# jaak-s/BayesianDataFusion.jl

Hardware: AMD Instinct MI355X
Metric: Gibbs sweeps/sec (both entities) + test RMSE, MovieLens-1M D=32 (higher is better)
Workload: dtype f64; 1 GPU; BPMF MovieLens-1M 6040x3952, 500209 training ratings (500000 held out), D=32, alpha=1.5, step = rows of both entities + hyperpriors + test prediction update (one native call); BEFORE the --warmup steps the engine's set-up runs 60 ms of full iterations whose results are discarded (device_warmup_ms); num_latent=32, burnin=5, psamples=1985, parallelism=1 GPU

## Files before the change

bayesiandatafusion.jl_amd/csrc/bdf_common.h:

```cpp
#pragma once
#include <map>
#include <array>
#include <algorithm>
#include <numeric>
#include <hip/hip_runtime.h>
#include <hip/hip_ext.h>
#include <cstdint>
#include <cstdio>
#include <cstdarg>
#include <cstring>
#include <vector>
#include "../../include/bdf.h"

void bdf_set_error(const char *fmt, ...);

#define BDF_HIP(expr)                                                                      \
    do {                                                                                   \
        hipError_t e__ = (expr);                                                           \
        if (e__ != hipSuccess) {                                                           \
            bdf_set_error("%s failed: %s (%s:%d)", #expr, hipGetErrorString(e__), __FILE__, __LINE__); \
            return BDF_ERR_HIP;                                                            \
        }                                                                                  \
    } while (0)

// ... 77 lines not shown
    bdf_rows_state *rows;
    double *norm_part;
};

int bdf_scratch(bdf_ctx *ctx, size_t bytes, void **out);
int bdf_scratch2(bdf_ctx *ctx, size_t bytes, void **out);
int bdf_sum_ranks_into(bdf_ctx *ctx, bdf_comm *comm, double *x, int64_t n, double *gather);
int bdf_sample_beta_rel_impl(bdf_ctx *ctx, bdf_comm *comm, const bdf_feat *fc, const bdf_pairs *train, int64_t first_obs, int D,
                             const double *const *factors, double mean_value, double alpha, const double *alpha_dev, double lambda_beta,
                             uint32_t rel_tag, double *beta_out, double *linear_out, double *rhs_out);
#define BDF_DRAWS_BATCH 8
int bdf_hyper_draws_batch(bdf_ctx *ctx, int D, int n, const int64_t *N, const double *nu, const uint32_t *entity_tag, double *const *draws_out);

struct bdf_mode_index {
    std::vector<int64_t> rowptr;
    std::vector<int64_t> rowids;
    std::vector<int32_t> order;
    int64_t *rowptr_dev;
    int32_t *colidx_dev;
    double  *vals_dev;
    int32_t *perm_dev;
    uint32_t *packed_dev;
    int32_t *order_dev;
    std::vector<int32_t> own_orig;
    std::vector<int32_t> own_pos;
    std::vector<int64_t> own_q;
    std::vector<int64_t> chunk_begin;
    int64_t own_nnz;
};

struct bdf_rel {
    bdf_ctx *ctx;
    uint64_t serial;
    int n_modes;
    int64_t dims[BDF_MAX_MODES];
    int64_t nnz;
    double value_mean;
    bdf_mode_index idx[BDF_MAX_MODES];
    int sharded;
    int rank, world, chunks;
    int64_t nint[BDF_MAX_MODES];
    int n_codes;
    double *table_dev;
};

struct bdf_pairs {
    bdf_ctx *ctx;
    int n_modes;
    int64_t n;
    int32_t *ids_dev;
    double *values_dev;
    double *avg_dev, *sq_dev;
    double count;
    const double *baseline_dev;
    int32_t *orig_dev;
    int sorted_mode;
    std::vector<int32_t> ids_host, orig_host;
    std::vector<double> values_host;
    void *auc_ws;
    int link;
    double link_r;
    double *lpd_dev;
    double lpd_draws;
    double *waic_dev;
    double waic_draws;
};

#define BDF_ORD_TABLE 17
#define BDF_ORD_CUR 0
#define BDF_ORD_PROP 17
#define BDF_ORD_JAC 34
#define BDF_ORD_SIGMA 35
#define BDF_ORD_PROPOSALS 36
#define BDF_ORD_ACCEPTS 37
#define BDF_ORD_LAST_S 38
#define BDF_ORD_ACCEPTED 39
#define BDF_ORD_VALID 40
#define BDF_ORD_LOGU 41
#define BDF_ORD_TRACE 48
#define BDF_ORD_MAX_TRACE ((int64_t)1 << 24)
struct bdf_ordinal {
    bdf_ctx *ctx;
    int K;
    int64_t capacity;
    int64_t adapt_steps;
    size_t state_doubles;
    double *state_dev;
    hipStream_t stream;
};

struct bdf_feat {
    bdf_ctx *ctx;
    int kind;
    int64_t m, n, nnz;
    double *dense_dev;
    int64_t *rowptr_dev; int32_t *colind_dev; double *rvals_dev;
    int64_t *colptr_dev; int32_t *rowind_dev; double *cvals_dev;
    int64_t *panel_fwd_dev; int n_panels_fwd;
    int64_t *panel_tr_dev; int n_panels_tr;
    double *FF_dev;
    int32_t *row_ids_dev;
    double *chol_ws;
    size_t chol_ws_doubles;
    void *gather_dev;
    size_t gather_bytes;
    bdf_feat *eig_Q;
    double *eig_s;
    double *eig_y;
    int eig_y_cols;
    bool eig_failed;
    bool FF_summed;
};
#define BDF_EIG_MAX 640

int bdf_chol_solve(bdf_ctx *ctx, bdf_feat *f, int D, const double *lambda_dev, const double *rhs, double *beta);

struct u32x4 { uint32_t x, y, z, w; };

__host__ __device__ __forceinline__ u32x4 philox4x32_10(u32x4 c, uint32_t k0, uint32_t k1)
{
#pragma unroll
    for (int r = 0; r < 10; r++) {
        uint64_t p0 = (uint64_t)0xD2511F53u * c.x;
        uint64_t p1 = (uint64_t)0xCD9E8D57u * c.z;
        u32x4 n;
        n.x = (uint32_t)(p1 >> 32) ^ c.y ^ k0;
        n.y = (uint32_t)p1;
        n.z = (uint32_t)(p0 >> 32) ^ c.w ^ k1;
        n.w = (uint32_t)p0;
        c = n;
        k0 += 0x9E3779B9u;
        k1 += 0xBB67AE85u;
    }
    return c;
}

__host__ __device__ __forceinline__ u32x4 bdf_draw(uint64_t seed, uint32_t sweep, uint32_t purpose, uint32_t entity,
                                          uint64_t row, uint32_t pair)
{
    u32x4 c;
    c.x = (uint32_t)row;
    c.y = (uint32_t)((row >> 32) & 0xffffu) | (pair << 16);
    c.z = sweep;
    c.w = (purpose << 24) | (entity & 0xffffffu);
    return philox4x32_10(c, (uint32_t)seed, (uint32_t)(seed >> 32));
}

__host__ __device__ __forceinline__ double bdf_u01(uint32_t lo, uint32_t hi)
{
    uint64_t x = ((uint64_t)hi << 32) | lo;
    return ((double)(x >> 11) + 0.5) * 0x1.0p-53;
}

__device__ __forceinline__ void bdf_sincos2pi(double u, double &s, double &c)
{
    const double q = rint(4.0 * u);
    const double x = 6.283185307179586476925286766559 * fma(q, -0.25, u);
    const double z = x * x;
    const double ps = fma(z, fma(z, fma(z, fma(z, fma(z, 1.58969099521155010221e-10, -2.50507602534068634195e-08),
                                                   2.75573137070700676789e-06), -1.98412698298579493134e-04),
                                     8.33333333332248946124e-03), -1.66666666666666324348e-01);
    const double pc = fma(z, fma(z, fma(z, fma(z, fma(z, -1.13596475577881948265e-11, 2.08757232129817482790e-09),
                                                   -2.75573143513906633035e-07), 2.48015872894767294178e-05),
                                     -1.38888888888741095749e-03), 4.16666666666666019037e-02);
    const double sx = fma(x * z, ps, x);
    const double cx = fma(z * z, pc, fma(z, -0.5, 1.0));
    const int iq = (int)q & 3;
    const double sa = (iq & 1) ? cx : sx, ca = (iq & 1) ? sx : cx;
    s = (iq & 2) ? -sa : sa;
    c = (iq == 1 || iq == 2) ? -ca : ca;
}

__device__ __forceinline__ double bdf_log01(double x)
{
    int k;
    double m = frexp(x, &k);
    if (m < 0.70710678118654752440) { m *= 2.0; k -= 1; }
    const double f = m - 1.0, dk = (double)k;
    const double s = f / (2.0 + f), z = s * s, w = z * z;
    const double t1 = w * fma(w, fma(w, 1.531383769920937332e-01, 2.222219843214978396e-01), 3.999999999940941908e-01);
    const double t2 = z * fma(w, fma(w, fma(w, 1.479819860511658591e-01, 1.818357216161805012e-01), 2.857142874366239149e-01),
                              6.666666666666735130e-01);
    const double R = t2 + t1, hfsq = 0.5 * f * f;
    return dk * 6.93147180369123816490e-01 - ((hfsq - fma(s, hfsq + R, dk * 1.90821492927058770002e-10)) - f);
}

__device__ __forceinline__ double bdf_normal(uint64_t seed, uint32_t sweep, uint32_t purpose, uint32_t entity,
                                    uint64_t row, int n)
{
    u32x4 o = bdf_draw(seed, sweep, purpose, entity, row, (uint32_t)(n >> 1));
    double u1 = bdf_u01(o.x, o.y), u2 = bdf_u01(o.z, o.w);
    double r = sqrt(-2.0 * bdf_log01(u1));
    double s, c;
    bdf_sincos2pi(u2, s, c);
    return (n & 1) ? r * s : r * c;
}

__device__ __forceinline__ void bdf_normal_pair(uint64_t seed, uint32_t sweep, uint32_t purpose, uint32_t entity,
                                       uint64_t row, uint32_t pair, double &z0, double &z1)
{
    u32x4 o = bdf_draw(seed, sweep, purpose, entity, row, pair);
    double u1 = bdf_u01(o.x, o.y), u2 = bdf_u01(o.z, o.w);
    double r = sqrt(-2.0 * bdf_log01(u1));
    double s, c;
    bdf_sincos2pi(u2, s, c);
    z0 = r * c;
    z1 = r * s;
}

__device__ __forceinline__ double bdf_uniform(uint64_t seed, uint32_t sweep, uint32_t purpose, uint32_t entity,
                                     uint64_t row, uint32_t pair)
{
    u32x4 o = bdf_draw(seed, sweep, purpose, entity, row, pair);
    return bdf_u01(o.x, o.y);
}

__device__ __forceinline__ double bdf_gamma_on(uint32_t p_normal, uint32_t p_uniform, uint64_t seed, uint32_t sweep, uint32_t entity,
                                               uint64_t g, double a)
{
    double boost = 1.0;
    if (a < 1.0) {
        boost = pow(bdf_uniform(seed, sweep, p_uniform, entity, g, 0xffffu), 1.0 / a);
        a += 1.0;
    }
    double d = a - 1.0 / 3.0, c = 1.0 / sqrt(9.0 * d);
    for (uint32_t t = 0; t < 256; t++) {
        double x = bdf_normal(seed, sweep, p_normal, entity, g, (int)(2 * t));
        double v = 1.0 + c * x;
        if (v <= 0.0) continue;
        v = v * v * v;
        double u = bdf_uniform(seed, sweep, p_uniform, entity, g, t);
        if (u < 1.0 - 0.0331 * (x * x) * (x * x)) return boost * d * v;
        if (log(u) < 0.5 * x * x + d * (1.0 - v + log(v))) return boost * d * v;
    }
    return boost * d;
}

__device__ __forceinline__ double bdf_gamma(uint64_t seed, uint32_t sweep, uint32_t entity, uint64_t g, double a)
{
    return bdf_gamma_on(BDF_P_GAMMA_N, BDF_P_GAMMA_U, seed, sweep, entity, g, a);
}

__device__ __forceinline__ double readlane_f64(double v, int lane)
{
    int lo = __builtin_amdgcn_readlane(__double2loint(v), lane);
    int hi = __builtin_amdgcn_readlane(__double2hiint(v), lane);
    return __hiloint2double(hi, lo);
}

#define BDF_DONE_SHARDS 64
#define BDF_DONE_STRIDE 16

int bdf_predict_plain(bdf_ctx *ctx, const bdf_pairs *p, int D, const double *const *factors, double mean_value, double *out);
int bdf_predict_link(bdf_ctx *ctx, const bdf_pairs *p, int D, const double *const *factors, double mean_value, const double *linear,
                     double *out, int phase, double count, double clamp_lo, double clamp_hi, double class_cut, double *stats_out);
int bdf_predict_link_pg(bdf_ctx *ctx, const bdf_pairs *p, int D, const double *const *factors, double mean_value, const double *linear,
                        double *out, int phase, double count, double clamp_lo, double clamp_hi, double class_cut, double *stats_out);
```

bayesiandatafusion.jl_amd/csrc/k_predict.hip:

```cpp
#include "bdf_common.h"
#include "predict.h"
#include <algorithm>
#include <cstdlib>

namespace {

template <int NM, int VEC, int NC>
__global__ __launch_bounds__(256) void k_predict(PredArgs a)
{
    const int tid = threadIdx.x, sub = tid & 7;
    double st[4] = {0.0, 0.0, 0.0, 0.0};
    const int64_t ngroups = (int64_t)gridDim.x * 32, ntrips = (a.n + 7) / 8;
    constexpr int BATCH = (VEC == 1) ? 2 : (NC * NM <= 3 ? 4 : 2);
    for (int64_t trip = (int64_t)blockIdx.x * 32 + tid / 8; trip < ntrips; trip += ngroups) {
        const int64_t p0 = trip * 8;
        PairState ps;
        pair_load(a, p0 + sub, ps);
        int32_t my[NM];
#pragma unroll
        for (int k = 0; k < NM; k++) my[k] = a.ids[(int64_t)k * a.n + ps.pm];
        double keep = 0.0;
#pragma unroll
        for (int u0 = 0; u0 < 8; u0 += BATCH) {
            if (p0 + u0 >= a.n) break;
// ... 134 lines not shown
}

namespace {
struct PredAllArgs {
    int D, n_modes;
    int64_t dims[BDF_MAX_MODES];
    const double *fac[BDF_MAX_MODES];
    double mean;
    double *out;
    int64_t rest;
};
__global__ __launch_bounds__(256) void k_predict_all(PredAllArgs a)
{
    __shared__ double u[16][BDF_MAX_D + 1];
    const int tx = threadIdx.x & 15, ty = threadIdx.x >> 4;
    const int64_t i0 = (int64_t)blockIdx.y * 16, c = (int64_t)blockIdx.x * 16 + tx;
    for (int e = threadIdx.x; e < 16 * a.D; e += 256) {
        const int r = e / a.D, d = e - r * a.D;
        u[r][d] = i0 + r < a.dims[0] ? a.fac[0][(i0 + r) * a.D + d] : 0.0;
    }
    __syncthreads();
    if (c >= a.rest || i0 + ty >= a.dims[0]) return;
    const double *row[BDF_MAX_MODES];
    int64_t q = c;
#pragma unroll
    for (int k = BDF_MAX_MODES - 1; k >= 1; k--)
        if (k < a.n_modes) { row[k] = a.fac[k] + (q % a.dims[k]) * a.D; q /= a.dims[k]; }
    double s = 0.0;
    for (int d = 0; d < a.D; d++) {
        double pr = u[ty][d];
#pragma unroll
        for (int k = 1; k < BDF_MAX_MODES; k++)
            if (k < a.n_modes) pr *= row[k][d];
        s += pr;
    }
    a.out[(i0 + ty) * a.rest + c] = s + a.mean;
}
}

extern "C" int bdf_predict_all(bdf_ctx *ctx, int n_modes, const int64_t *dims, int D, const double *const *factors,
                               double mean_value, double *out)
{
    BDF_REQUIRE(ctx && dims && factors && out, BDF_ERR_ARG, "bdf_predict_all: NULL argument");
    BDF_REQUIRE(n_modes >= 2 && n_modes <= BDF_MAX_MODES, BDF_ERR_ARG, "bdf_predict_all: n_modes=%d must be in 2..%d", n_modes, BDF_MAX_MODES);
    BDF_REQUIRE(D >= 1 && D <= BDF_MAX_D, BDF_ERR_ARG, "bdf_predict_all: num_latent=%d must be in 1..%d", D, BDF_MAX_D);
    PredAllArgs a;
    memset(&a, 0, sizeof(a));
    a.D = D; a.n_modes = n_modes; a.mean = mean_value; a.out = out; a.rest = 1;
    for (int k = 0; k < n_modes; k++) {
        BDF_REQUIRE(dims[k] >= 0 && factors[k] != nullptr, BDF_ERR_ARG, "bdf_predict_all: dims[%d] < 0 or factors[%d] NULL", k, k);
        a.dims[k] = dims[k]; a.fac[k] = factors[k];
        if (k >= 1) a.rest *= dims[k];
    }
    if (a.dims[0] == 0 || a.rest == 0) return BDF_OK;
    const int64_t gx = (a.rest + 15) / 16, gy = (a.dims[0] + 15) / 16;
    BDF_REQUIRE(gx < (int64_t)0x7fffffff && gy <= 65535 * (int64_t)1024, BDF_ERR_BOUNDS, "bdf_predict_all: %lld x %lld cells are too many for one launch",
                (long long)a.dims[0], (long long)a.rest);
    BDF_HIP(hipSetDevice(ctx->device));
    for (int64_t y0 = 0; y0 < gy; y0 += 65535) {
        PredAllArgs b = a;
        const int64_t ny = std::min<int64_t>(65535, gy - y0);
        b.fac[0] = a.fac[0] + y0 * 16 * D;
        b.dims[0] = std::min<int64_t>(a.dims[0] - y0 * 16, ny * 16);
        b.out = a.out + y0 * 16 * a.rest;
        hipLaunchKernelGGL(k_predict_all, dim3((unsigned)gx, (unsigned)ny), dim3(256), 0, ctx->stream, b);
    }
    BDF_HIP(hipGetLastError());
    return BDF_OK;
}

extern "C" int bdf_pairs_create(bdf_ctx *ctx, int n_modes, int64_t n, const void *ids, int id_bytes,
                                const double *values, bdf_pairs **out)
{
    BDF_REQUIRE(ctx && out, BDF_ERR_ARG, "bdf_pairs_create: NULL argument");
    BDF_REQUIRE(n_modes >= 2 && n_modes <= BDF_MAX_MODES, BDF_ERR_ARG, "bdf_pairs_create: n_modes=%d must be in 2..%d", n_modes, BDF_MAX_MODES);
    BDF_REQUIRE(id_bytes == 4 || id_bytes == 8, BDF_ERR_ARG, "bdf_pairs_create: id_bytes must be 4 or 8");
    BDF_REQUIRE(n >= 0 && (n == 0 || (ids && values)), BDF_ERR_ARG, "bdf_pairs_create: ids/values NULL");
    BDF_HIP(hipSetDevice(ctx->device));
    std::vector<int32_t> h((size_t)n * n_modes);
    for (size_t q = 0; q < h.size(); q++) {
        int64_t v = id_bytes == 8 ? ((const int64_t *)ids)[q] : (int64_t)((const int32_t *)ids)[q];
        BDF_REQUIRE(v >= 1 && v < (int64_t)0x7fffffff, BDF_ERR_BOUNDS, "bdf_pairs_create: id %lld out of range", (long long)v);
        h[q] = (int32_t)(v - 1);
    }
    bdf_pairs *p = new bdf_pairs();
    p->ctx = ctx; p->n_modes = n_modes; p->n = n; p->count = 0.0; p->baseline_dev = nullptr; p->orig_dev = nullptr; p->sorted_mode = -1;
    p->ids_dev = nullptr; p->values_dev = nullptr; p->avg_dev = nullptr; p->sq_dev = nullptr; p->auc_ws = nullptr; p->link = 0; p->link_r = 0.0;
    p->lpd_dev = nullptr; p->lpd_draws = 0.0; p->waic_dev = nullptr; p->waic_draws = 0.0;
    struct Guard { bdf_pairs *p; ~Guard() { if (p) bdf_pairs_destroy(p); } } guard{p};
    p->ids_host = h;
    p->values_host.assign(values, values + (n ? n : 0));
    size_t nb = std::max<size_t>((size_t)n * sizeof(double), 8);
    BDF_HIP(hipMalloc((void **)&p->ids_dev, std::max<size_t>(h.size() * sizeof(int32_t), 8)));
    BDF_HIP(hipMalloc((void **)&p->values_dev, nb));
    BDF_HIP(hipMalloc((void **)&p->avg_dev, nb));
    BDF_HIP(hipMalloc((void **)&p->sq_dev, nb));
    if (n) {
        BDF_HIP(hipMemcpy(p->ids_dev, h.data(), h.size() * sizeof(int32_t), hipMemcpyHostToDevice));
        BDF_HIP(hipMemcpy(p->values_dev, values, (size_t)n * sizeof(double), hipMemcpyHostToDevice));
    }
    BDF_HIP(hipMemsetAsync(p->avg_dev, 0, nb, ctx->stream));
    BDF_HIP(hipMemsetAsync(p->sq_dev, 0, nb, ctx->stream));
    BDF_HIP(hipStreamSynchronize(ctx->stream));
    guard.p = nullptr;
    *out = p;
    return BDF_OK;
}

extern "C" int bdf_pairs_destroy(bdf_pairs *p)
{
    if (!p) return BDF_OK;
    hipSetDevice(p->ctx->device);
    hipStreamSynchronize(p->ctx->stream);
    hipFree(p->ids_dev); hipFree(p->values_dev); hipFree(p->avg_dev); hipFree(p->sq_dev);
    if (p->orig_dev) hipFree(p->orig_dev);
    if (p->auc_ws) hipFree(p->auc_ws);
    if (p->lpd_dev) hipFree(p->lpd_dev);
    if (p->waic_dev) hipFree(p->waic_dev);
    delete p;
    return BDF_OK;
}

extern "C" int bdf_predict(bdf_ctx *ctx, const bdf_pairs *p, int D, const double *const *factors,
                           double mean_value, double *out)
{
    PredArgs a;
    int rc = fill("bdf_predict", ctx, p, D, factors, a);
    if (rc) return rc;
    BDF_REQUIRE(out != nullptr, BDF_ERR_ARG, "bdf_predict: out is NULL");
    a.mean = mean_value; a.out = out;
    return p->link ? bdf_predict_link(ctx, p, D, factors, mean_value, nullptr, out, -1, 0.0, 1.0, 0.0, 0.0, nullptr) : launch_predict(ctx, a);
}

int bdf_predict_plain(bdf_ctx *ctx, const bdf_pairs *p, int D, const double *const *factors, double mean_value, double *out)
{
    PredArgs a;
    int rc = fill("bdf_predict", ctx, p, D, factors, a);
    if (rc) return rc;
    a.mean = mean_value; a.linear = nullptr; a.out = out;
    return launch_predict(ctx, a);
}

extern "C" int bdf_predict_update(bdf_ctx *ctx, bdf_pairs *p, int D, const double *const *factors,
                                  double mean_value, int phase, double clamp_lo, double clamp_hi,
                                  double class_cut, double *stats_out)
{
    PredArgs a;
    int rc = fill("bdf_predict_update", ctx, p, D, factors, a);
    if (rc) return rc;
    BDF_REQUIRE(stats_out != nullptr, BDF_ERR_ARG, "bdf_predict_update: stats_out is NULL");
    BDF_REQUIRE(phase >= 0 && phase <= 2, BDF_ERR_ARG, "bdf_predict_update: phase must be 0, 1 or 2");
    a.mean = mean_value; a.avg = p->avg_dev; a.sq = p->sq_dev; a.phase = phase; a.count = p->count;
    a.clamp_lo = clamp_lo; a.clamp_hi = clamp_hi; a.cut = class_cut; a.stats = stats_out;
    rc = p->link ? bdf_predict_link(ctx, p, D, factors, mean_value, nullptr, nullptr, phase, p->count, clamp_lo, clamp_hi, class_cut, stats_out)
                 : launch_predict(ctx, a);
    if (rc) return rc;
    if (phase == 1) p->count = 1.0;
    else if (phase == 2) p->count += 1.0;
    return BDF_OK;
}

extern "C" int bdf_predict_sse(bdf_ctx *ctx, const bdf_pairs *p, int D, const double *const *factors, double mean_value,
                               const double *linear_values, double *stats_out)
{
    PredArgs a;
    int rc = fill("bdf_predict_sse", ctx, p, D, factors, a);
    if (rc) return rc;
    BDF_REQUIRE(stats_out != nullptr, BDF_ERR_ARG, "bdf_predict_sse: stats_out is NULL");
    a.mean = mean_value; if (linear_values) a.linear = linear_values; a.phase = 3; a.count = 0.0;
    a.clamp_lo = 1.0; a.clamp_hi = 0.0; a.cut = 0.0; a.stats = stats_out;
    if (p->link) return bdf_predict_link(ctx, p, D, factors, mean_value, linear_values, nullptr, 3, 0.0, 1.0, 0.0, 0.0, stats_out);
    return launch_predict(ctx, a);
}

extern "C" int bdf_pairs_sort(bdf_pairs *p, int mode)
{
    BDF_REQUIRE(p != nullptr, BDF_ERR_ARG, "bdf_pairs_sort: NULL argument");
    BDF_REQUIRE(mode >= 0 && mode < p->n_modes, BDF_ERR_ARG, "bdf_pairs_sort: mode %d out of range", mode);
    BDF_REQUIRE(p->count == 0.0 && p->orig_dev == nullptr, BDF_ERR_ARG, "bdf_pairs_sort: the pairs already hold prediction state or are sorted");
    const int64_t n = p->n;
    if (n == 0) return BDF_OK;
    BDF_HIP(hipSetDevice(p->ctx->device));
    std::vector<int32_t> perm((size_t)n);
    for (int64_t i = 0; i < n; i++) perm[(size_t)i] = (int32_t)i;
    const int32_t *key = p->ids_host.data() + (size_t)mode * n;
    std::stable_sort(perm.begin(), perm.end(), [key](int32_t x, int32_t y) { return key[x] < key[y]; });
    std::vector<int32_t> ids((size_t)n * p->n_modes);
    std::vector<double> vals((size_t)n);
    for (int k = 0; k < p->n_modes; k++)
        for (int64_t i = 0; i < n; i++) ids[(size_t)k * n + i] = p->ids_host[(size_t)k * n + perm[(size_t)i]];
    for (int64_t i = 0; i < n; i++) vals[(size_t)i] = p->values_host[(size_t)perm[(size_t)i]];
    BDF_HIP(hipStreamSynchronize(p->ctx->stream));
    BDF_HIP(hipMemcpy(p->ids_dev, ids.data(), ids.size() * sizeof(int32_t), hipMemcpyHostToDevice));
    BDF_HIP(hipMemcpy(p->values_dev, vals.data(), vals.size() * sizeof(double), hipMemcpyHostToDevice));
    BDF_HIP(hipMalloc((void **)&p->orig_dev, (size_t)n * sizeof(int32_t)));
    BDF_HIP(hipMemcpy(p->orig_dev, perm.data(), (size_t)n * sizeof(int32_t), hipMemcpyHostToDevice));
    p->orig_host = perm;
    p->sorted_mode = mode;
    return BDF_OK;
}

extern "C" int bdf_pairs_order(const bdf_pairs *p, int64_t *orig_host)
{
    BDF_REQUIRE(p && orig_host, BDF_ERR_ARG, "bdf_pairs_order: NULL argument");
    for (int64_t i = 0; i < p->n; i++) orig_host[i] = p->orig_host.empty() ? i : (int64_t)p->orig_host[(size_t)i];
    return BDF_OK;
}

extern "C" int bdf_pairs_set_baseline(bdf_pairs *p, const double *baseline)
{
    BDF_REQUIRE(p != nullptr, BDF_ERR_ARG, "bdf_pairs_set_baseline: NULL argument");
    p->baseline_dev = baseline;
    return BDF_OK;
}

extern "C" int bdf_pairs_set_link(bdf_pairs *p, int link)
{
    BDF_REQUIRE(p != nullptr, BDF_ERR_ARG, "bdf_pairs_set_link: NULL argument");
    BDF_REQUIRE(link == 0 || link == 1, BDF_ERR_ARG, "bdf_pairs_set_link: link=%d must be 0 (identity) or 1 (probit)", link);
    p->link = link;
    return BDF_OK;
}

extern "C" int bdf_pairs_set_logistic_link(bdf_pairs *p)
{
    BDF_REQUIRE(p != nullptr, BDF_ERR_ARG, "bdf_pairs_set_logistic_link: NULL argument");
    p->link = 2;
    return BDF_OK;
}

extern "C" int bdf_pairs_set_count_link(bdf_pairs *p, double r)
{
    BDF_REQUIRE(p != nullptr, BDF_ERR_ARG, "bdf_pairs_set_count_link: NULL argument");
    BDF_REQUIRE(r >= 1.0 && r <= 2147483648.0 && r == std::floor(r), BDF_ERR_ARG, "bdf_pairs_set_count_link: r=%g must be an integer, at least 1", r);
    p->link = 3;
    p->link_r = r;
    return BDF_OK;
}

extern "C" int bdf_pairs_state(const bdf_pairs *p, double **avg, double **sq, int64_t *n)
{
    BDF_REQUIRE(p && avg && sq && n, BDF_ERR_ARG, "bdf_pairs_state: NULL argument");
    *avg = p->avg_dev; *sq = p->sq_dev; *n = p->n;
    return BDF_OK;
}
```

bayesiandatafusion.jl_amd/csrc/k_rows_col.hip:

```cpp
#include "rows.h"
#include "dpp_rows32.h"
#include <algorithm>

#ifndef BDF_COL_WAVES
#define BDF_COL_WAVES 2
#endif
#define COL_PSZ 800

#ifdef BDF_K1_STAMPS
#define CSTAMP_DECL unsigned long long st_t = __builtin_amdgcn_s_memtime(), st_acc = 0, st_mid = 0, st_prior = 0, st_fin = 0, st_rng = 0, st_steps = 0, st_rounds = 0, st_parts = 0, st_fins = 0, st_folds = 0; const unsigned long long st_begin = st_t
#define CSTAMP(x) do { const unsigned long long now_ = __builtin_amdgcn_s_memtime(); x += now_ - st_t; st_t = now_; } while (0)
#else
#define CSTAMP_DECL do { } while (0)
#define CSTAMP(x) do { } while (0)
#endif

namespace {

template <int DR, int K>
__device__ __forceinline__ void col_obs(double (&A0)[33], double (&A1)[33], double v0, double v1, double r)
{
    col_rank1<DR, 0>(A0, A1, v0, v1);
    fm1_run<K>(A0[32], r, v0);
    fm1_run<K>(A1[32], r, v1);
}

__device__ __forceinline__ double col_ld(__amdgpu_buffer_rsrc_t rs, uint32_t off)
{
    typedef unsigned u2v __attribute__((ext_vector_type(2)));
    const u2v x = __builtin_amdgcn_raw_buffer_load_b64(rs, (int)off, 0, 0);
    return __hiloint2double((int)x.y, (int)x.x);
}

template <bool FULL, int K0>
__device__ __forceinline__ void col_gather4(double (&b)[4][2], __amdgpu_buffer_rsrc_t rs, uint32_t idw, uint32_t rowb, uint32_t eo, bool ok1)
{
#pragma unroll
    for (int q = 0; q < 4; q++) {
        uint32_t id;
        if (q == 0) id = row_bcast_u32<K0>(idw); else if (q == 1) id = row_bcast_u32<K0 + 1>(idw);
        else if (q == 2) id = row_bcast_u32<K0 + 2>(idw); else id = row_bcast_u32<K0 + 3>(idw);
        if constexpr (FULL) {
            const uint32_t base = id + eo;
            b[q][1] = col_ld(rs, base);
            b[q][0] = col_ld(rs, base + 128u);
        } else {
            const uint32_t base = id + eo;
            b[q][0] = col_ld(rs, base);
            b[q][1] = col_ld(rs, ok1 ? base - 128u : 0xffffffffu);
        }
    }
}
template <int DR, int K0>
__device__ __forceinline__ void col_compute4(double (&A0)[33], double (&A1)[33], const double (&b)[4][2], double r)
{
    col_obs<DR, K0>(A0, A1, b[0][0], b[0][1], r);
    col_obs<DR, K0 + 1>(A0, A1, b[1][0], b[1][1], r);
    col_obs<DR, K0 + 2>(A0, A1, b[2][0], b[2][1], r);
    col_obs<DR, K0 + 3>(A0, A1, b[3][0], b[3][1], r);
}

template <int X>
__device__ __forceinline__ void col_fold(double (&A0)[33], double (&A1)[33], double m)
{
#pragma unroll
    for (int i = 0; i < 33; i++) A0[i] = fma(__shfl_xor(A0[i], X), m, A0[i]);
#pragma unroll
    for (int i = 16; i < 33; i++) A1[i] = fma(__shfl_xor(A1[i], X), m, A1[i]);
}

template <int E0, int E1, bool ADD>
__device__ __forceinline__ void col_slot_load(double (&A0)[33], double (&A1)[33], const double *src, double m)
{
#pragma unroll
    for (int e = E0; e < E1; e++) {
        const double v = src[e * 16];
        double &d = e < 33 ? A0[e] : A1[e - 17];
        if (ADD) d = fma(v, m, d); else d = v * m;
    }
}

__device__ __forceinline__ void col_prior_dma(const double *image, unsigned lds_dst, int lane)
{
    const void *sbase = (const void *)(((uint64_t)(uint32_t)__builtin_amdgcn_readfirstlane((int)((uint64_t)image >> 32)) << 32) |
                                       (uint32_t)__builtin_amdgcn_readfirstlane((int)(uint32_t)(uint64_t)image));
#pragma unroll
    for (int k = 0; k < 6; k++) {
        const unsigned voff = (unsigned)k * 1024u + (unsigned)lane * 16u;
        unsigned keep;
        asm volatile("s_mov_b32 %0, m0\n\ts_mov_b32 m0, %2\n\ts_nop 0\n\tglobal_load_lds_dwordx4 %1, %3 sc1\n\ts_mov_b32 m0, %0"
                     : "=&s"(keep) : "v"(voff), "s"(lds_dst + (unsigned)k * 1024u), "s"(sbase) : "memory");
    }
}
template <int S, int I, int DR>
__device__ __forceinline__ void col_prior_lds(double (&A)[33], const double *img, double alpha, int j)
{
    if constexpr (I < DR) {
        A[I] = fma(alpha, A[I], img[sys_off<S, I>(j)]);
        col_prior_lds<S, I + 1, DR>(A, img, alpha, j);
    }
}

template <int DR, bool FULL>
__global__ __launch_bounds__(64, BDF_COL_WAVES) void k_rows_col(SampleArgs a_in, ColPlanDev p_in, uint32_t fac_bytes)
{
    __shared__ __attribute__((aligned(16))) double lds[4 * 272 + 768];
    const int w = blockIdx.x;
    if (w >= p_in.n_waves) return;
    const int r_end = p_in.wave_round[w + 1];
    if (a_in.span && threadIdx.x == 0) atomicMin(a_in.span + 2 * (w & 63), (unsigned long long)__builtin_amdgcn_s_memrealtime());
    CSTAMP_DECL;
#pragma nounroll
    for (int rd = p_in.wave_round[w]; rd < r_end; rd++) {
    int zero = 0, lane = threadIdx.x;
    asm volatile("" : "+s"(zero), "+v"(lane));
    const SampleArgs &a = (&a_in)[zero];
    const ColPlanDev &p = (&p_in)[zero];
    const int j = lane & 15, g = lane >> 4;
    const TermDev &T = a.t[0];
    const int D = FULL ? 32 : a.D;
    const int ec0 = D - 1 - j, ec1 = D - 17 - j;
    const int n0 = ec0, n1 = ec1 >= 0 ? ec1 : 0;
    const bool ok1 = ec1 >= 0;
    const uint32_t rowb = (uint32_t)D * 8u;
    const uint32_t eo = FULL ? (uint32_t)ec1 * 8u : (uint32_t)ec0 * 8u;
    const __amdgpu_buffer_rsrc_t rs = __builtin_amdgcn_make_buffer_rsrc((void *)T.fac[0], 0, (int)fac_bytes, 0x00020000);
    const bool coded = T.packed != nullptr;
    const double mean = T.mean;
    {
        const ColJob jb = p.jobs[(int64_t)rd * 4 + g];
        const bool live = jb.row >= 0;
        const int n = live ? jb.count : 0;
        const unsigned lds_img = (unsigned)__builtin_amdgcn_readfirstlane((int)(unsigned)(size_t)(__attribute__((address_space(3))) double *)(lds + 4 * 272));
        bool have_prior = true;
        if (a.ready) have_prior = __builtin_amdgcn_readfirstlane((int)((int32_t)(__hip_atomic_load(a.ready, __ATOMIC_RELAXED, __HIP_MEMORY_SCOPE_AGENT) - a.ready_want) >= 0)) != 0;
        if (have_prior) col_prior_dma(a.prior_c, lds_img, lane);
        double A0[33], A1[33];
#pragma unroll
        for (int i = 0; i < 33; i++) { A0[i] = 0.0; A1[i] = 0.0; }
        int nmax = n;
        nmax = max(nmax, __shfl_xor(nmax, 16));
        nmax = max(nmax, __shfl_xor(nmax, 32));
        nmax = __builtin_amdgcn_readfirstlane(nmax);
        if (nmax > 0) {
            const uint32_t *packed = coded ? T.packed + jb.q_begin : nullptr;
            const int32_t *colidx = T.colidx + jb.q_begin;
            const double *vals = T.vals + jb.q_begin;
            const double *table = T.table;
#define COL_CHUNK(c0, IDW, R)                                                                     \
            {                                                                                     \
                const int o_ = (c0) + j;                                                          \
                IDW = 0xffffffu; R = 0.0;                                                         \
                if (o_ < n) {                                                                     \
                    if (coded) { const uint32_t pw_ = packed[o_]; IDW = pw_; R = table[pw_ >> 24] - mean; } \
                    else { IDW = (uint32_t)colidx[o_]; R = vals[o_] - mean; }                     \
                }                                                                                 \
                IDW = __umul24(IDW, rowb);       \
            }
            uint32_t idw_c, idw_n;
            double r_c, r_n;
            COL_CHUNK(0, idw_c, r_c)
            double ba[4][2], bb[4][2];
            col_gather4<FULL, 0>(ba, rs, idw_c, rowb, eo, ok1);
            for (int c0 = 0;; c0 += 16) {
                COL_CHUNK(c0 + 16, idw_n, r_n)
                col_gather4<FULL, 4>(bb, rs, idw_c, rowb, eo, ok1);
                __builtin_amdgcn_sched_barrier(0);
                col_compute4<DR, 0>(A0, A1, ba, r_c);
                if (c0 + 4 >= nmax) break;
                col_gather4<FULL, 8>(ba, rs, idw_c, rowb, eo, ok1);
                __builtin_amdgcn_sched_barrier(0);
                col_compute4<DR, 4>(A0, A1, bb, r_c);
                if (c0 + 8 >= nmax) break;
                col_gather4<FULL, 12>(bb, rs, idw_c, rowb, eo, ok1);
                __builtin_amdgcn_sched_barrier(0);
                col_compute4<DR, 8>(A0, A1, ba, r_c);
                if (c0 + 12 >= nmax) break;
                col_gather4<FULL, 0>(ba, rs, idw_n, rowb, eo, ok1);
                __builtin_amdgcn_sched_barrier(0);
                col_compute4<DR, 12>(A0, A1, bb, r_c);
                if (c0 + 16 >= nmax) break;
                idw_c = idw_n; r_c = r_n;
            }
#undef COL_CHUNK
        }
#ifdef BDF_K1_STAMPS
        asm volatile("s_nop 0" :: "v"(A0[0]), "v"(A0[32]), "v"(A1[31]));
        st_steps += (unsigned long long)nmax; st_rounds++;
#endif
        CSTAMP(st_acc);
        const unsigned fl = (unsigned)jb.flags;
        if (__builtin_amdgcn_readfirstlane((int)(__ballot((fl & COLF_PAIR) != 0) != 0ull))) {
#ifdef BDF_K1_STAMPS
            st_folds++;
#endif
            col_fold<16>(A0, A1, (fl & COLF_PAIR) ? 1.0 : 0.0);
            if (__builtin_amdgcn_readfirstlane((int)(__ballot((fl & COLF_QUAD) != 0) != 0ull)))
                col_fold<32>(A0, A1, (fl & COLF_QUAD) ? 1.0 : 0.0);
        }
        if (__builtin_amdgcn_readfirstlane((int)(fl & COLF_MULTI))) {
            const int srow = __builtin_amdgcn_readfirstlane(jb.srow);
            double *dst = p.partials + (int64_t)__builtin_amdgcn_readfirstlane(jb.slot) * COL_PSZ + j;
            if (g == 0) {
#pragma unroll
                for (int e = 0; e < 33; e++) __hip_atomic_store(dst + e * 16, A0[e], __ATOMIC_RELAXED, __HIP_MEMORY_SCOPE_AGENT);
#pragma unroll
                for (int e = 33; e < 50; e++) __hip_atomic_store(dst + e * 16, A1[e - 17], __ATOMIC_RELAXED, __HIP_MEMORY_SCOPE_AGENT);
            }
            const ColSplit sr = p.rows[srow];
            asm volatile("s_waitcnt vmcnt(0)" ::: "memory");
            int old = 0;
            if (lane == 0) old = __hip_atomic_fetch_add(p.arrived + srow, 1, __ATOMIC_RELAXED, __HIP_MEMORY_SCOPE_AGENT);
            old = __builtin_amdgcn_readfirstlane(old);
#ifdef BDF_K1_STAMPS
            st_parts++;
            if (old == sr.n_slots - 1) st_fins++;
#endif
            if (old != sr.n_slots - 1) { CSTAMP(st_mid); continue; }
            __builtin_amdgcn_fence(__ATOMIC_ACQUIRE, "agent");
            asm volatile("s_waitcnt vmcnt(0)" ::: "memory");
            if (lane == 0) p.arrived[srow] = 0;
            const double *src = p.partials + (int64_t)sr.slot_begin * COL_PSZ + j;
            col_slot_load<0, 50, false>(A0, A1, src + (int64_t)(g < sr.n_slots ? g : 0) * COL_PSZ, g < sr.n_slots ? 1.0 : 0.0);
            for (int s0 = 4; s0 < sr.n_slots; s0 += 4) {
                const bool on = s0 + g < sr.n_slots;
                const double *sp = src + (int64_t)(on ? s0 + g : 0) * COL_PSZ;
                const double m = on ? 1.0 : 0.0;
                col_slot_load<0, 16, true>(A0, A1, sp, m);
                asm volatile("" ::: "memory");
                col_slot_load<16, 33, true>(A0, A1, sp, m);
                asm volatile("" ::: "memory");
                col_slot_load<33, 50, true>(A0, A1, sp, m);
                asm volatile("" ::: "memory");
            }
            col_fold<16>(A0, A1, 1.0);
            col_fold<32>(A0, A1, 1.0);
        }
        CSTAMP(st_mid);
        double z0 = 0.0, z1 = 0.0;
        {
            double ze = 0.0, zo = 0.0;
            if (live && 2 * j < D) bdf_normal_pair(a.seed, a.sweep, BDF_P_ROW, a.entity_tag, (uint64_t)(uint32_t)jb.orig, (uint32_t)j, ze, zo);
            const int base = lane & 48;
            const double ze0 = __shfl(ze, base + (n0 >> 1)), zo0 = __shfl(zo, base + (n0 >> 1));
            const double ze1 = __shfl(ze, base + (n1 >> 1)), zo1 = __shfl(zo, base + (n1 >> 1));
            z0 = (n0 & 1) ? zo0 : ze0;
            z1 = ok1 ? ((n1 & 1) ? zo1 : ze1) : 0.0;
        }
        asm volatile("" ::: "memory");
        CSTAMP(st_rng);
        {
            double *tl = lds + g * 272;
#pragma unroll
            for (int r = 0; r < 16; r++) tl[r * 17 + j] = A0[16 + r];
            wave_sync();
#pragma unroll
            for (int i = 0; i < 16; i++) A1[i] = tl[j * 17 + i];
            wave_sync();
        }
        CSTAMP(st_mid);
        const double alpha = term_alpha(T);
        if (!have_prior) {
            int spins = 0;
            while ((int32_t)(__hip_atomic_load(a.ready, __ATOMIC_RELAXED, __HIP_MEMORY_SCOPE_AGENT) - a.ready_want) < 0) {
                __builtin_amdgcn_s_sleep(16);
                if (++spins > (1 << 22)) { if (lane == 0) atomicOr_system(a.flag, 16); break; }
            }
            col_prior_dma(a.prior_c, lds_img, lane);
        }
        {
            const double *pb = a.prior_b + (a.mu_is_matrix && live ? (int64_t)jb.row * D : 0);
            const double b0 = __hip_atomic_load(pb + n0, __ATOMIC_RELAXED, __HIP_MEMORY_SCOPE_AGENT);
            const double b1 = __hip_atomic_load(pb + n1, __ATOMIC_RELAXED, __HIP_MEMORY_SCOPE_AGENT);
            asm volatile("s_waitcnt vmcnt(0)" ::: "memory");
            wave_sync();
            const double *img = lds + 4 * 272;
            col_prior_lds<0, 0, DR>(A0, img, alpha, j);
            col_prior_lds<1, 0, DR>(A1, img, alpha, j);
            A0[32] = fma(alpha, A0[32], b0);
            A1[32] = ok1 ? fma(alpha, A1[32], b1) : 0.0;
            wave_sync();
        }
#ifdef BDF_K1_STAMPS
        asm volatile("s_nop 0" :: "v"(A0[0]), "v"(A0[31]), "v"(A1[0]), "v"(A1[31]));
#endif
        CSTAMP(st_prior);
        double d0 = 1.0, d1 = 1.0;
        fin_factor<DR, 0>(A0, A1, d0, d1, j);
        const bool lead = live && (fl & COLF_LEADER);
        if (lead && (!(d0 > 0.0) || (ok1 && !(d1 > 0.0)))) atomicOr_system(a.flag, 1);
        const double rd0 = fast_rcp(d0), rd1 = fast_rcp(d1);
        double y0 = fma(z0, fast_rsqrt(d0), A0[32] * rd0), y1 = fma(z1, fast_rsqrt(d1), A1[32] * rd1);
        fin_backward<DR - 1>(A0, A1, y0, y1, rd0, rd1, j);
        if (lead) __hip_atomic_store(a.out + ((int64_t)jb.row * D + ec0), y0, __ATOMIC_RELAXED, __HIP_MEMORY_SCOPE_AGENT);
        if (lead && ok1) __hip_atomic_store(a.out + ((int64_t)jb.row * D + ec1), y1, __ATOMIC_RELAXED, __HIP_MEMORY_SCOPE_AGENT);
        CSTAMP(st_fin);
    }
    }
    if (a_in.done) {
        asm volatile("s_waitcnt vmcnt(0)" ::: "memory");
        if (threadIdx.x == 0) __hip_atomic_fetch_add(a_in.done + BDF_DONE_STRIDE * (w & (BDF_DONE_SHARDS - 1)), 1u, __ATOMIC_RELAXED, __HIP_MEMORY_SCOPE_AGENT);
    }
    if (a_in.span && threadIdx.x == 0) atomicMax(a_in.span + 2 * (w & 63) + 1, (unsigned long long)__builtin_amdgcn_s_memrealtime());
#ifdef BDF_K1_STAMPS
    if (threadIdx.x == 0 && a_in.b_dump && w < 65536) {
        unsigned long long *d = (unsigned long long *)a_in.b_dump + (size_t)w * 16;
        d[0] = st_begin; d[8] = st_t; d[6] = st_rounds; d[7] = st_steps;
        d[1] = st_parts; d[2] = st_fins; d[3] = st_folds;
        d[11] = st_rng; d[12] = st_acc; d[13] = st_mid; d[14] = st_prior; d[15] = st_fin;
        d[9] = __builtin_amdgcn_s_getreg((4 - 1) << 11 | 0 << 6 | 4) | ((unsigned long long)__builtin_amdgcn_s_getreg((32 - 1) << 11 | 0 << 6 | 4));
        d[10] = __builtin_amdgcn_s_getreg((4 - 1) << 11 | 0 << 6 | 20);
    }
#endif
}

#define COL_C_OBS 56.0
#define COL_C_FIN 1460.0
#define COL_C_FOLD 180.0
#define COL_C_PART 700.0

struct Round { ColJob job[4]; double cost; };

ColJob idle_job() { return ColJob{-1, 0, 0, 0, -1, 0, 0}; }

}

int bdf_col_plan_build(bdf_ctx *ctx, const std::vector<bdf_row_ref> &rows, int T, int64_t slots, bdf_col_plan &plan)
{
    std::vector<Round> rounds;
    std::vector<ColSplit> splits;
    struct Unit { int32_t row, orig; int64_t qb; int32_t n; };
    std::vector<Unit> singles, pairs;
    int32_t n_slots_total = 0;
    auto quad_round = [&](const bdf_row_ref &rr, int64_t b0, int64_t b1, int32_t srow, int32_t slot, double fin_share) {
        Round R;
        const int64_t m = b1 - b0;
        int32_t lmax = 0;
        for (int q = 0; q < 4; q++) {
            const int64_t p0 = b0 + m * q / 4, p1 = b0 + m * (q + 1) / 4;
            R.job[q] = ColJob{rr.out, rr.orig, rr.qb + p0, (int32_t)(p1 - p0), srow, slot,
                              (int32_t)(COLF_PAIR | COLF_QUAD | (q == 0 ? COLF_LEADER : 0) | (srow >= 0 ? COLF_MULTI : 0))};
            lmax = std::max(lmax, (int32_t)(p1 - p0));
        }
        constexpr double part_extra = 3000.0;
        R.cost = COL_C_OBS * lmax + 2 * COL_C_FOLD + (srow >= 0 ? COL_C_PART + fin_share + part_extra : COL_C_FIN);
        rounds.push_back(R);
    };
    for (const bdf_row_ref &rr : rows) {
        const int64_t n = rr.cnt;
        if (n <= T) singles.push_back(Unit{rr.out, rr.orig, rr.qb, (int32_t)n});
        else if (n <= 2 * (int64_t)T) pairs.push_back(Unit{rr.out, rr.orig, rr.qb, (int32_t)n});
        else if (n <= 4 * (int64_t)T) quad_round(rr, 0, n, -1, 0, 0.0);
        else {
            const int64_t W = (n + 4 * (int64_t)T - 1) / (4 * (int64_t)T);
            BDF_REQUIRE(W < (1 << 20), BDF_ERR_ARG, "bdf_sample_rows: a row of %lld observations", (long long)n);
            const int32_t srow = (int32_t)splits.size();
            splits.push_back(ColSplit{n_slots_total, (int32_t)W});
            const double share = (COL_C_FIN + 2 * COL_C_FOLD + 60.0 * (double)((W + 3) / 4)) / (double)W;
            for (int64_t q = 0; q < W; q++) quad_round(rr, n * q / W, n * (q + 1) / W, srow, n_slots_total + (int32_t)q, share);
            n_slots_total += (int32_t)W;
        }
    }
    auto by_len = [](const Unit &x, const Unit &y) { return x.n > y.n; };
    std::stable_sort(pairs.begin(), pairs.end(), by_len);
    std::stable_sort(singles.begin(), singles.end(), by_len);
    auto pair_jobs = [](const Unit &u, ColJob *dst) {
        const int32_t h = u.n / 2;
        dst[0] = ColJob{u.row, u.orig, u.qb, h, -1, 0, COLF_PAIR | COLF_LEADER};
        dst[1] = ColJob{u.row, u.orig, u.qb + h, u.n - h, -1, 0, COLF_PAIR};
    };
    size_t si = 0;
    for (size_t pi = 0; pi < pairs.size(); pi += 2) {
        Round R;
        pair_jobs(pairs[pi], R.job);
        int32_t lmax = pairs[pi].n - pairs[pi].n / 2;
        if (pi + 1 < pairs.size()) pair_jobs(pairs[pi + 1], R.job + 2);
        else {
            for (int q = 2; q < 4; q++) {
                if (si < singles.size()) {
                    const Unit &u = singles[si++];
                    R.job[q] = ColJob{u.row, u.orig, u.qb, u.n, -1, 0, COLF_LEADER};
                    lmax = std::max(lmax, u.n);
                } else R.job[q] = idle_job();
            }
        }
        R.cost = COL_C_OBS * lmax + COL_C_FOLD + COL_C_FIN;
        rounds.push_back(R);
    }
    for (; si < singles.size(); si += 4) {
        Round R;
        for (int q = 0; q < 4; q++) {
            if (si + q < singles.size()) {
                const Unit &u = singles[si + q];
                R.job[q] = ColJob{u.row, u.orig, u.qb, u.n, -1, 0, COLF_LEADER};
            } else R.job[q] = idle_job();
// ... 80 lines not shown
```

Before: 12310 sweeps/s.

## Add sorted-run test prediction kernel and cap column-kernel VGPRs with SGPR constants

Adds a new prediction-update kernel for sorted two-mode test pairs. Each 8-lane group handles a run of 16 consecutive pairs and reloads the sorted-side factor row only when its id changes, which cuts redundant gathers. Separately, the row-sampling column kernel gets an explicit VGPR cap, and its RNG polynomial constants are forced into scalar registers through a template coefficient policy, to relieve vector register pressure. The cap risks spills, and the new path assumes sorted ids with D a multiple of 4 and at most 32.

Measured after the change: 12740 sweeps/s (median of 6 runs). +3.4%, better.

```diff
diff --git a/bayesiandatafusion.jl_amd/csrc/bdf_common.h b/bayesiandatafusion.jl_amd/csrc/bdf_common.h
--- a/bayesiandatafusion.jl_amd/csrc/bdf_common.h
+++ b/bayesiandatafusion.jl_amd/csrc/bdf_common.h
@@ -253,17 +253,20 @@
     return ((double)(x >> 11) + 0.5) * 0x1.0p-53;
 }
 
+struct BdfLiteral { static __device__ __forceinline__ double c(double x) { return x; } };
+
+template <class KC = BdfLiteral>
 __device__ __forceinline__ void bdf_sincos2pi(double u, double &s, double &c)
 {
     const double q = rint(4.0 * u);
-    const double x = 6.283185307179586476925286766559 * fma(q, -0.25, u);
+    const double x = KC::c(6.283185307179586476925286766559) * fma(q, -0.25, u);
     const double z = x * x;
-    const double ps = fma(z, fma(z, fma(z, fma(z, fma(z, 1.58969099521155010221e-10, -2.50507602534068634195e-08),
-                                                   2.75573137070700676789e-06), -1.98412698298579493134e-04),
-                                     8.33333333332248946124e-03), -1.66666666666666324348e-01);
-    const double pc = fma(z, fma(z, fma(z, fma(z, fma(z, -1.13596475577881948265e-11, 2.08757232129817482790e-09),
-                                                   -2.75573143513906633035e-07), 2.48015872894767294178e-05),
-                                     -1.38888888888741095749e-03), 4.16666666666666019037e-02);
+    const double ps = fma(z, fma(z, fma(z, fma(z, fma(z, KC::c(1.58969099521155010221e-10), KC::c(-2.50507602534068634195e-08)),
+                                                   KC::c(2.75573137070700676789e-06)), KC::c(-1.98412698298579493134e-04)),
+                                     KC::c(8.33333333332248946124e-03)), KC::c(-1.66666666666666324348e-01));
+    const double pc = fma(z, fma(z, fma(z, fma(z, fma(z, KC::c(-1.13596475577881948265e-11), KC::c(2.08757232129817482790e-09)),
+                                                   KC::c(-2.75573143513906633035e-07)), KC::c(2.48015872894767294178e-05)),
+                                     KC::c(-1.38888888888741095749e-03)), KC::c(4.16666666666666019037e-02));
     const double sx = fma(x * z, ps, x);
     const double cx = fma(z * z, pc, fma(z, -0.5, 1.0));
     const int iq = (int)q & 3;
@@ -272,18 +275,19 @@
     c = (iq == 1 || iq == 2) ? -ca : ca;
 }
 
+template <class KC = BdfLiteral>
 __device__ __forceinline__ double bdf_log01(double x)
 {
     int k;
     double m = frexp(x, &k);
-    if (m < 0.70710678118654752440) { m *= 2.0; k -= 1; }
+    if (m < KC::c(0.70710678118654752440)) { m *= 2.0; k -= 1; }
     const double f = m - 1.0, dk = (double)k;
     const double s = f / (2.0 + f), z = s * s, w = z * z;
-    const double t1 = w * fma(w, fma(w, 1.531383769920937332e-01, 2.222219843214978396e-01), 3.999999999940941908e-01);
-    const double t2 = z * fma(w, fma(w, fma(w, 1.479819860511658591e-01, 1.818357216161805012e-01), 2.857142874366239149e-01),
-                              6.666666666666735130e-01);
+    const double t1 = w * fma(w, fma(w, KC::c(1.531383769920937332e-01), KC::c(2.222219843214978396e-01)), KC::c(3.999999999940941908e-01));
+    const double t2 = z * fma(w, fma(w, fma(w, KC::c(1.479819860511658591e-01), KC::c(1.818357216161805012e-01)), KC::c(2.857142874366239149e-01)),
+                              KC::c(6.666666666666735130e-01));
     const double R = t2 + t1, hfsq = 0.5 * f * f;
-    return dk * 6.93147180369123816490e-01 - ((hfsq - fma(s, hfsq + R, dk * 1.90821492927058770002e-10)) - f);
+    return dk * KC::c(6.93147180369123816490e-01) - ((hfsq - fma(s, hfsq + R, dk * KC::c(1.90821492927058770002e-10))) - f);
 }
 
 __device__ __forceinline__ double bdf_normal(uint64_t seed, uint32_t sweep, uint32_t purpose, uint32_t entity,
@@ -297,14 +301,15 @@
     return (n & 1) ? r * s : r * c;
 }
 
+template <class KC = BdfLiteral>
 __device__ __forceinline__ void bdf_normal_pair(uint64_t seed, uint32_t sweep, uint32_t purpose, uint32_t entity,
                                        uint64_t row, uint32_t pair, double &z0, double &z1)
 {
     u32x4 o = bdf_draw(seed, sweep, purpose, entity, row, pair);
     double u1 = bdf_u01(o.x, o.y), u2 = bdf_u01(o.z, o.w);
-    double r = sqrt(-2.0 * bdf_log01(u1));
+    double r = sqrt(-2.0 * bdf_log01<KC>(u1));
     double s, c;
-    bdf_sincos2pi(u2, s, c);
+    bdf_sincos2pi<KC>(u2, s, c);
     z0 = r * c;
     z1 = r * s;
 }
@@ -353,6 +358,8 @@
 #define BDF_DONE_STRIDE 16
 
 int bdf_predict_plain(bdf_ctx *ctx, const bdf_pairs *p, int D, const double *const *factors, double mean_value, double *out);
+int bdf_update_runs(bdf_ctx *ctx, const bdf_pairs *p, int D, const double *const *factors, double mean_value, int phase, double count,
+                    double clamp_lo, double clamp_hi, double class_cut, double *stats_out);
 int bdf_predict_link(bdf_ctx *ctx, const bdf_pairs *p, int D, const double *const *factors, double mean_value, const double *linear,
                      double *out, int phase, double count, double clamp_lo, double clamp_hi, double class_cut, double *stats_out);
 int bdf_predict_link_pg(bdf_ctx *ctx, const bdf_pairs *p, int D, const double *const *factors, double mean_value, const double *linear,
diff --git a/bayesiandatafusion.jl_amd/csrc/k_predict.hip b/bayesiandatafusion.jl_amd/csrc/k_predict.hip
--- a/bayesiandatafusion.jl_amd/csrc/k_predict.hip
+++ b/bayesiandatafusion.jl_amd/csrc/k_predict.hip
@@ -310,7 +310,9 @@
     BDF_REQUIRE(phase >= 0 && phase <= 2, BDF_ERR_ARG, "bdf_predict_update: phase must be 0, 1 or 2");
     a.mean = mean_value; a.avg = p->avg_dev; a.sq = p->sq_dev; a.phase = phase; a.count = p->count;
     a.clamp_lo = clamp_lo; a.clamp_hi = clamp_hi; a.cut = class_cut; a.stats = stats_out;
+    const bool runs = a.sorted_mode >= 0 && a.n_modes == 2 && (a.D & 3) == 0 && a.D <= 32 && a.linear == nullptr;
     rc = p->link ? bdf_predict_link(ctx, p, D, factors, mean_value, nullptr, nullptr, phase, p->count, clamp_lo, clamp_hi, class_cut, stats_out)
+         : runs  ? bdf_update_runs(ctx, p, D, factors, mean_value, phase, p->count, clamp_lo, clamp_hi, class_cut, stats_out)
                  : launch_predict(ctx, a);
     if (rc) return rc;
     if (phase == 1) p->count = 1.0;
diff --git a/bayesiandatafusion.jl_amd/csrc/k_rows_col.hip b/bayesiandatafusion.jl_amd/csrc/k_rows_col.hip
--- a/bayesiandatafusion.jl_amd/csrc/k_rows_col.hip
+++ b/bayesiandatafusion.jl_amd/csrc/k_rows_col.hip
@@ -5,6 +5,7 @@
 #ifndef BDF_COL_WAVES
 #define BDF_COL_WAVES 2
 #endif
+#define COL_VGPR_HALF 104
 #define COL_PSZ 800
 
 #ifdef BDF_K1_STAMPS
@@ -16,6 +17,8 @@
 #endif
 
 namespace {
+
+struct ColCoef { static __device__ __forceinline__ double c(double x) { asm volatile("" : "+s"(x)); return x; } };
 
 template <int DR, int K>
 __device__ __forceinline__ void col_obs(double (&A0)[33], double (&A1)[33], double v0, double v1, double r)
@@ -102,7 +105,7 @@
 }
 
 template <int DR, bool FULL>
-__global__ __launch_bounds__(64, BDF_COL_WAVES) void k_rows_col(SampleArgs a_in, ColPlanDev p_in, uint32_t fac_bytes)
+__global__ __launch_bounds__(64, BDF_COL_WAVES) __attribute__((amdgpu_num_vgpr(COL_VGPR_HALF))) void k_rows_col(SampleArgs a_in, ColPlanDev p_in, uint32_t fac_bytes)
 {
     __shared__ __attribute__((aligned(16))) double lds[4 * 272 + 768];
     const int w = blockIdx.x;
@@ -240,7 +243,7 @@
         double z0 = 0.0, z1 = 0.0;
         {
             double ze = 0.0, zo = 0.0;
-            if (live && 2 * j < D) bdf_normal_pair(a.seed, a.sweep, BDF_P_ROW, a.entity_tag, (uint64_t)(uint32_t)jb.orig, (uint32_t)j, ze, zo);
+            if (live && 2 * j < D) bdf_normal_pair<ColCoef>(a.seed, a.sweep, BDF_P_ROW, a.entity_tag, (uint64_t)(uint32_t)jb.orig, (uint32_t)j, ze, zo);
             const int base = lane & 48;
             const double ze0 = __shfl(ze, base + (n0 >> 1)), zo0 = __shfl(zo, base + (n0 >> 1));
             const double ze1 = __shfl(ze, base + (n1 >> 1)), zo1 = __shfl(zo, base + (n1 >> 1));
diff --git a/bayesiandatafusion.jl_amd/csrc/k_update_runs.hip b/bayesiandatafusion.jl_amd/csrc/k_update_runs.hip
--- /dev/null
+++ b/bayesiandatafusion.jl_amd/csrc/k_update_runs.hip
@@ -0,0 +1,76 @@
+#include "bdf_common.h"
+#include "predict.h"
+
+namespace {
+
+constexpr int RUN = 16;
+constexpr int NB = 4;
+
+__global__ __launch_bounds__(256) void k_update_runs(PredArgs a)
+{
+    const int tid = threadIdx.x, sub = tid & 7;
+    const int ks = a.sorted_mode, ko = 1 - ks;
+    const int32_t *ids_s = a.ids + (int64_t)ks * a.n, *ids_o = a.ids + (int64_t)ko * a.n;
+    const double *fs = a.fac[ks], *fo = a.fac[ko];
+    const bool live = sub * 4 < a.D;
+    const int eoff = live ? sub * 4 : 0;
+    const int64_t p0 = ((int64_t)blockIdx.x * 32 + tid / 8) * RUN;
+    int32_t cur = -1;
+    double4 srow = {0.0, 0.0, 0.0, 0.0};
+    double keep[2] = {0.0, 0.0};
+#pragma unroll
+    for (int q = 0; q < 2; q++) {
+        if (p0 + 8 * q >= a.n) break;
+        const int64_t pm = p0 + 8 * q + sub < a.n ? p0 + 8 * q + sub : a.n - 1;
+        const int32_t my_s = ids_s[pm], my_o = ids_o[pm];
+#pragma unroll
+        for (int u0 = 0; u0 < 8; u0 += NB) {
+            double4 orow[NB];
+#pragma unroll
+            for (int u = 0; u < NB; u++) orow[u] = *(const double4 *)(fo + (int64_t)__shfl(my_o, u0 + u, 8) * a.D + eoff);
+#pragma unroll
+            for (int u = 0; u < NB; u++) {
+                const int32_t is = __shfl(my_s, u0 + u, 8);
+                if (is != cur) { srow = *(const double4 *)(fs + (int64_t)is * a.D + eoff); cur = is; }
+                double s = live ? (srow.x * orow[u].x + srow.y * orow[u].y) + (srow.z * orow[u].z + srow.w * orow[u].w) : 0.0;
+                s += __shfl_xor(s, 4); s += __shfl_xor(s, 2); s += __shfl_xor(s, 1);
+                if (sub == u0 + u) keep[q] = s;
+            }
+        }
+    }
+    __builtin_amdgcn_sched_barrier(0);
+    double st[4] = {0.0, 0.0, 0.0, 0.0};
+#pragma unroll
+    for (int q = 0; q < 2; q++) {
+        PairState ps;
+        const int64_t p = p0 + 8 * q + sub;
+        ps.ok = p < a.n;
+        ps.pm = ps.ok ? p : a.n - 1;
+        ps.po = ps.pm;
+        ps.base = a.mean;
+        ps.y = a.values[ps.pm];
+        ps.av = 0.0; ps.sv = 0.0;
+        if (a.phase == 2) { ps.av = a.avg[ps.pm]; ps.sv = a.sq[ps.pm]; }
+        pair_finish(a, ps, keep[q], st);
+    }
+    block_stats(a, st);
+}
+
+}
+
+int bdf_update_runs(bdf_ctx *ctx, const bdf_pairs *p, int D, const double *const *factors, double mean_value, int phase, double count,
+                    double clamp_lo, double clamp_hi, double class_cut, double *stats_out)
+{
+    PredArgs a;
+    int rc = fill("bdf_predict_update", ctx, p, D, factors, a);
+    if (rc) return rc;
+    BDF_REQUIRE(a.sorted_mode >= 0 && a.n_modes == 2 && (D & 3) == 0 && D <= 32 && a.linear == nullptr && phase >= 0 && phase <= 2,
+                BDF_ERR_ARG, "bdf_update_runs: not the sorted two-mode update");
+    if (a.n == 0) return BDF_OK;
+    a.mean = mean_value; a.avg = p->avg_dev; a.sq = p->sq_dev; a.phase = phase; a.count = count;
+    a.clamp_lo = clamp_lo; a.clamp_hi = clamp_hi; a.cut = class_cut; a.stats = stats_out;
+    a.orig = nullptr; a.out = nullptr;
+    const int nblocks = (int)((a.n + 32 * RUN - 1) / (32 * RUN));
+    return launch_reduced(ctx, nblocks, a.partial, a.stats,
+                          [&] { hipLaunchKernelGGL(k_update_runs, dim3(nblocks), dim3(256), 0, ctx->stream, a); });
+}
```
